# SFGLab/MultiMM

Hardware: NVIDIA B200
Metric: force_evals_per_s (higher is better)
Workload: dtype f32

## Files before the change

multimm_b200/csrc/mmm_api.cu:

```cuda
#include <math.h>
#include <string.h>

#include <algorithm>
#include <new>

#include "mmm_internal.cuh"

int mmm_launch_dots_decide(mmm_system* h);

static thread_local std::string g_create_error;
static void free_scratch(mmm_system* h);

int mmm_fail(mmm_system* h, int code, const std::string& msg) {
  if (h) h->err = msg;
  else g_create_error = msg;
  return code;
}

#define REQUIRE(h, cond, msg) \
  do { if (!(cond)) return mmm_fail((h), MMM_ERR_ARG, (msg)); } while (0)

static void derive_pair_params(mmm_system* h) {
  PairParams& p = h->pp;
  p.ev_pref = p.ev_form == MMM_EV_POWERLAW ? p.ev_eps * powf(p.ev_sigma, p.ev_power) : 0.0f;
  const float rc = p.scb_form >= 0 ? p.scb_rc : p.cob_rc;
  if (rc > 0.0f) {
    p.g_c = -1.4426950408889634f / (2.0f * rc * rc);
    p.g_inv_rc2 = 1.0f / (rc * rc);
    p.rg2 = 2.0f * rc * rc * 26.0f * 0.6931471805599453f;
  } else {
    p.g_c = 0.0f; p.g_inv_rc2 = 0.0f; p.rg2 = 0.0f;
  }
  p.cutoff2 = (float)h->cutoff * (float)h->cutoff;
}

extern "C" {

int mmm_abi_version(void) { return MMM_ABI_VERSION; }

const char* mmm_last_error(mmm_handle h) { return h ? h->err.c_str() : g_create_error.c_str(); }

int mmm_create(int device, int64_t n_beads, mmm_handle* out) {
  if (!out) return mmm_fail(nullptr, MMM_ERR_ARG, "mmm_create: out is NULL");
  *out = nullptr;
  if (n_beads < 2 || n_beads > (int64_t)1 << 24)
    return mmm_fail(nullptr, MMM_ERR_ARG, "mmm_create: n_beads must be in [2, 2^24]");
  int ndev = 0;
  cudaError_t e = cudaGetDeviceCount(&ndev);
  if (e != cudaSuccess || ndev == 0)
    return mmm_fail(nullptr, MMM_ERR_CUDA,
                    std::string("CUDA error: no usable device (") + cudaGetErrorString(e) +
                        "); this engine has no CPU fallback");
  if (device < 0 || device >= ndev) return mmm_fail(nullptr, MMM_ERR_ARG, "mmm_create: device index out of range");
  cudaDeviceProp prop;
  e = cudaGetDeviceProperties(&prop, device);
  if (e != cudaSuccess) return mmm_fail(nullptr, MMM_ERR_CUDA, std::string("CUDA error: ") + cudaGetErrorString(e));
  if (prop.major != 10)
    return mmm_fail(nullptr, MMM_ERR_CUDA,
                    "CUDA error: device is not sm_100 (B200); the kernels are built for sm_100a only");
  mmm_system* h = new (std::nothrow) mmm_system();
  if (!h) return mmm_fail(nullptr, MMM_ERR_NOMEM, "out of host memory");
  h->device = device;
  h->n = n_beads;
  h->npad = (n_beads + MMM_PAD_TO - 1) / MMM_PAD_TO * MMM_PAD_TO;
  h->ntiles = h->npad / MMM_TILE;
  h->sm_count = prop.multiProcessorCount;
  h->pp.ev_form = h->pp.cob_form = h->pp.scb_form = h->pp.chb_form = MMM_FORM_OFF;
  h->ep.sc_form = h->ep.lam_form = h->ep.cf_form = MMM_FORM_OFF;
  h->n_red_blocks = (int)((n_beads + MMM_ASM_BLOCK - 1) / MMM_ASM_BLOCK);
  h->n_dot_blocks = std::min(h->n_red_blocks, 2 * h->sm_count);
  int rc = MMM_OK;
  auto fail = [&](int code) { g_create_error = h->err; mmm_destroy(h); return code; };
  if (cudaSetDevice(device) != cudaSuccess) return fail(mmm_fail(h, MMM_ERR_CUDA, "CUDA error: cudaSetDevice"));
  if (cudaStreamCreateWithFlags(&h->stream, cudaStreamNonBlocking) != cudaSuccess)
    return fail(mmm_fail(h, MMM_ERR_CUDA, "CUDA error: cudaStreamCreate"));
  cudaEventCreate(&h->ev_a);
  cudaEventCreate(&h->ev_b);
  const size_t n3 = 3 * (size_t)n_beads;
  if ((rc = mmm_reserve(h, h->d_type, (size_t)h->npad, "bead types")) ||
      (rc = mmm_reserve(h, h->d_cstr, (size_t)n_beads, "chromosome strengths")) ||
      (rc = mmm_reserve(h, h->d_s, (size_t)n_beads, "compartment labels")) ||
      (rc = mmm_reserve(h, h->d_x, n3, "positions")) ||
      (rc = mmm_reserve(h, h->d_center, 3, "centre")) ||
      (rc = mmm_reserve(h, h->d_pos4, (size_t)h->npad, "FP32 positions")) ||
      (rc = mmm_reserve(h, h->d_soa, 3 * (size_t)h->npad, "FP32 coordinate planes")) ||
      (rc = mmm_reserve(h, h->d_tiles, (size_t)h->ntiles, "tile boxes")) ||
      (rc = mmm_reserve(h, h->d_g, n3, "gradient")) ||
      (rc = mmm_reserve(h, h->d_counter, 4, "work counters")) ||
      (rc = mmm_reserve(h, h->d_epart, (size_t)h->n_red_blocks * 6, "energy partials")) ||
      (rc = mmm_reserve(h, h->d_dpart, (size_t)h->n_red_blocks * MMM_NDOT, "dot partials")) ||
      (rc = mmm_reserve(h, h->d_eterms, MMM_NUM_TERMS, "energy terms")) ||
      (rc = mmm_reserve(h, h->d_lb, 1, "L-BFGS state")))
    return fail(rc);
  if (cudaMallocHost((void**)&h->h_done, 64) != cudaSuccess)
    return fail(mmm_fail(h, MMM_ERR_NOMEM, "CUDA error: cudaMallocHost"));
  cudaMemsetAsync(h->d_cstr, 0, sizeof(double) * n_beads, h->stream);
  cudaMemsetAsync(h->d_s, 0, n_beads, h->stream);
  cudaMemsetAsync(h->d_lb, 0, sizeof(LbfgsState), h->stream);
  std::vector<int> ty((size_t)h->npad);
  for (int64_t i = 0; i < h->npad; ++i)
    ty[i] = i < n_beads ? mmm_pack_type(0, 0) : mmm_pack_type(0, MMM_PAD_CHROM + (int)(i - n_beads));
  cudaMemcpyAsync(h->d_type, ty.data(), sizeof(int) * ty.size(), cudaMemcpyHostToDevice, h->stream);
  if (cudaStreamSynchronize(h->stream) != cudaSuccess)
    return fail(mmm_fail(h, MMM_ERR_CUDA, "CUDA error: initialisation copies failed"));
  h->types_dirty = false;
  *out = h;
  return MMM_OK;
}

int mmm_destroy(mmm_handle h) {
  if (!h) return MMM_OK;
  cudaSetDevice(h->device);
  if (h->stream) cudaStreamSynchronize(h->stream);
  mmm_dist_destroy(h);
  if (h->h_done) cudaFreeHost(h->h_done);
  for (cudaEvent_t e : h->ev_pool) cudaEventDestroy(e);
  for (cudaEvent_t e : {h->ev_a, h->ev_b, h->ev_c0, h->ev_c1, h->ct_ev0, h->ct_ev1, h->dm_ev0, h->dm_ev1,
                        h->sp_ev0, h->sp_ev1, h->lp_ev0, h->lp_ev1})
    if (e) cudaEventDestroy(e);
  if (h->stream) cudaStreamDestroy(h->stream);
  delete h;
  return MMM_OK;
}

static int check_pairs(mmm_system* h, const int32_t* i, const int32_t* j, int64_t cnt, const char* what) {
  for (int64_t q = 0; q < cnt; ++q)
    if (i[q] < 0 || j[q] < 0 || i[q] >= h->n || j[q] >= h->n || i[q] == j[q])
      return mmm_fail(h, MMM_ERR_ARG, std::string(what) + ": bead index out of range or degenerate");
  return MMM_OK;
}

int mmm_set_bonds(mmm_handle h, const int32_t* i, const int32_t* j, const double* r0, const double* k,
                  int64_t n_bonds) {
  if (!h) return MMM_ERR_ARG;
  REQUIRE(h, n_bonds >= 0 && (n_bonds == 0 || (i && j && r0 && k)), "mmm_set_bonds: NULL array");
  int rc = check_pairs(h, i, j, n_bonds, "mmm_set_bonds");
  if (rc) return rc;
  h->h_bond_i.assign(i, i + n_bonds); h->h_bond_j.assign(j, j + n_bonds);
  h->h_bond_r0.assign(r0, r0 + n_bonds); h->h_bond_k.assign(k, k + n_bonds);
  h->n_bonds = n_bonds;
  h->topo_dirty = true;
  return MMM_OK;
}

int mmm_set_loops(mmm_handle h, const int32_t* i, const int32_t* j, const double* r0, const double* k,
                  int64_t n_loops, int form) {
  if (!h) return MMM_ERR_ARG;
  REQUIRE(h, form >= MMM_LOOP_HARMONIC && form <= MMM_LOOP_GAUSSIAN_TETHER, "Unknown loop force type");
  REQUIRE(h, n_loops >= 0 && (n_loops == 0 || (i && j && r0 && k)), "mmm_set_loops: NULL array");
  int rc = check_pairs(h, i, j, n_loops, "mmm_set_loops");
  if (rc) return rc;
  h->h_loop_i.assign(i, i + n_loops); h->h_loop_j.assign(j, j + n_loops);
  h->h_loop_r0.assign(r0, r0 + n_loops); h->h_loop_k.assign(k, k + n_loops);
  h->n_loops = n_loops;
  h->loop_form = form;
  h->topo_dirty = true;
  return MMM_OK;
}

int mmm_set_angles(mmm_handle h, const int32_t* i, const int32_t* j, const int32_t* k, const double* theta0,
// ... 533 lines not shown
```

multimm_b200/csrc/mmm_internal.cuh:

```cuda
#pragma once

#include <cuda_runtime.h>
#include <stdint.h>

#include <string>
#include <vector>

#include "../../include/multimm_b200.h"

constexpr int MMM_TILE = 32;
constexpr int MMM_IBLOCK = 256;
constexpr int MMM_STAGE = 256;
constexpr int MMM_ASM_BLOCK = 128;
#ifndef MMM_LBFGS_M_VALUE
#define MMM_LBFGS_M_VALUE 6
#endif
constexpr int MMM_LBFGS_M = MMM_LBFGS_M_VALUE;
constexpr int MMM_NDOT = 6 * MMM_LBFGS_M + 7;
constexpr int MMM_PAD_TO = 512;
constexpr float MMM_PAD_COORD = 1.0e10f;
constexpr float MMM_PAD_STEP = 1.0e7f;
constexpr int MMM_PAD_CHROM = 0xFC00;

__host__ __device__ inline int mmm_pack_type(int s, int chrom) {
// ... 249 lines not shown
  cudaEvent_t dm_ev0 = nullptr, dm_ev1 = nullptr;

  bool sp_configured = false;
  double sp_rc = 0.0;
  int32_t sp_ct_bins = 0, sp_fine_bins = 0, sp_dm_bins = 0;
  DevBuf<int> d_sp_ct_bin, d_sp_fine_bin, d_sp_dm_bin;
  std::vector<int64_t> sp_dm_occ;
  int64_t sp_samples = 0;
  double sp_dm_bound = 0.0;
  float sp_ms = 0.f;
  cudaEvent_t sp_ev0 = nullptr, sp_ev1 = nullptr;
  DevBuf<unsigned long long> d_sp_map;
  DevBuf<unsigned long long> d_sp_sep;
  DevBuf<unsigned long long> d_sp_cnt;
  DevBuf<unsigned long long> d_sp_dist;
  DevBuf<long long> d_sp_tile, d_sp_table;
  DevBuf<unsigned long long> d_sp_keys[2];
  DevBuf<unsigned long long> d_sp_sval;
  DevBuf<unsigned long long> d_sp_acc_key[2], d_sp_acc_val[2];
  DevBuf<long long> d_sp_mpart;
  int64_t sp_fine_n = 0;

  bool lp_configured = false;
  double lp_rc = 0.0;
  int lp_w = 0;
  int64_t lp_rows = 0;
  int64_t lp_samples = 0;
  double lp_bound = 0.0;
  float lp_ms = 0.f;
  cudaEvent_t lp_ev0 = nullptr, lp_ev1 = nullptr;
  DevBuf<LoopRow> d_lp_row;
  DevBuf<unsigned long long> d_lp_sum;
};

struct CsSorted {
  long long keys = 0, entries = 0;
  int src = 0;
  unsigned long long cnt[2] = {0, 0};
};

int mmm_fail(mmm_system* h, int code, const std::string& msg);
#define MMM_CUDA(h, call)                                                                  \
  do {                                                                                     \
    cudaError_t _e = (call);                                                               \
    if (_e != cudaSuccess)                                                                 \
      return mmm_fail((h), MMM_ERR_CUDA,                                                   \
                      std::string("CUDA error: ") + cudaGetErrorString(_e) + " at " #call); \
  } while (0)

template <class T>
int mmm_reserve(mmm_system* h, DevBuf<T>& buf, size_t count, const char* what) {
  if (count <= buf.cap_) return MMM_OK;
  if (h && h->capturing)
    return mmm_fail(h, MMM_ERR_STATE, std::string("allocation of ") + what + " while a CUDA graph is captured");
  if (h && buf.p_) cudaStreamSynchronize(h->stream);
  buf.reset();
  cudaError_t e = cudaMalloc((void**)&buf.p_, count * sizeof(T));
  if (e != cudaSuccess) {
    buf.p_ = nullptr;
    return mmm_fail(h, MMM_ERR_NOMEM, std::string("CUDA error: ") + cudaGetErrorString(e) + " (cudaMalloc, " + what + ")");
  }
  buf.cap_ = count;
  return MMM_OK;
}

template <class T>
int mmm_upload(mmm_system* h, DevBuf<T>& buf, const std::vector<T>& v, const char* what) {
  if (v.empty()) {
    buf.reset();
    return MMM_OK;
  }
  int rc = mmm_reserve(h, buf, v.size(), what);
  if (rc) return rc;
  MMM_CUDA(h, cudaMemcpyAsync(buf, v.data(), v.size() * sizeof(T), cudaMemcpyHostToDevice, h->stream));
  MMM_CUDA(h, cudaStreamSynchronize(h->stream));
  return MMM_OK;
}

int mmm_launch_prepare(mmm_system* h, const int* d_skip);
int mmm_launch_hilbert(mmm_system* h, int p, double spacing, int32_t* d_ijk);
int mmm_launch_pair_exact(mmm_system* h, const int* d_skip, const PairParams* pp_override = nullptr);
bool mmm_pair_fast_path(const mmm_system* h);
bool mmm_pair_fast_path_pp(const PairParams& p);
bool mmm_pair_n3_eligible(const mmm_system* h);
bool mmm_pair_n3_generic(const mmm_system* h);
int mmm_n3_build_items(mmm_system* h, std::vector<int2>& items, bool chb_only);
int mmm_launch_pair_n3(mmm_system* h, const int* d_skip, bool chb_only = false);
int mmm_dist_allreduce(mmm_system* h);
void mmm_dist_destroy(mmm_system* h);
int mmm_launch_pair_n3_cut(mmm_system* h, const int* d_skip);
int mmm_cut_warp_build_items(mmm_system* h, std::vector<int2>& items);
int mmm_launch_pair_cutoff_n3(mmm_system* h, const int* d_skip);
int mmm_cutoff_resort_period();
int mmm_chb_clusters_build(mmm_system* h);
int mmm_chb_clusters_blocks(const mmm_system* h);
int mmm_launch_chb_clusters(mmm_system* h, const int* d_skip);
int mmm_launch_pair_cutoff(mmm_system* h, const int* d_skip);
int64_t mmm_cells_energy_slots(const mmm_system* h);
int mmm_upload_topology(mmm_system* h);
int mmm_upload_angles(mmm_system* h, const int32_t* ai, const int32_t* aj, const int32_t* ak,
                      const double* t0, const double* kt, int64_t na);
int mmm_launch_assemble(mmm_system* h, const int* d_skip);
int mmm_launch_finalize_energy(mmm_system* h);
int mmm_run_minimize(mmm_system* h, double tol, int64_t max_iter, mmm_min_report* out);

int mmm_contacts_dense_pass(mmm_system* h, double rc_nm, const int* d_bin, int32_t n_bins, unsigned long long* map,
                            unsigned long long* sep, unsigned long long* cnt, bool clear, cudaEvent_t ev0);
int mmm_contacts_sparse_pass(mmm_system* h, double rc_nm, const int* d_bin, int32_t n_bins, DevBuf<long long>& tile,
                             DevBuf<unsigned long long>* keys, DevBuf<long long>& table, unsigned long long* cnt,
                             cudaEvent_t ev0, cudaEvent_t ev1, CsSorted* out);
int mmm_contacts_fine_accumulate(mmm_system* h);
int mmm_contacts_fine_read(mmm_system* h, int32_t* rows_out, int32_t* cols_out, uint64_t* vals_out);
int mmm_distance_qmax(mmm_system* h, const char* who, double* dpad, double* qmax);
int mmm_distance_guard(mmm_system* h, const char* who, const std::vector<int64_t>& occ, double prior, double* bound);
int mmm_distance_pass(mmm_system* h, const int* d_bin, int32_t n_bins, unsigned long long* dmap,
                      unsigned long long* d2map, bool clear);

int mmm_evaluate(mmm_system* h, const int* d_skip);
```

multimm_b200/csrc/mmm_pair_n3.cu:

```cuda
#include <algorithm>

#include "mmm_internal.cuh"
#include "mmm_pairmath.cuh"

namespace {

constexpr int N3_THREADS = 256;
constexpr int N3_WARPS = N3_THREADS / 32;
constexpr int N3_IB = 512;
constexpr int N3_JB = 256;
constexpr int N3_STEPS = N3_JB / MMM_TILE;
constexpr double N3_FIXED = 16777216.0;
#ifndef N3_GROUP_UNROLL
#define N3_GROUP_UNROLL 2
#endif
constexpr int kGroupUnroll = N3_GROUP_UNROLL;
#ifndef N3_USE_F32X2
#define N3_USE_F32X2 1
#endif
#ifndef N3_PACKED_NEAR
#define N3_PACKED_NEAR 1
#endif
#ifndef N3_MIN_BLOCKS
#define N3_MIN_BLOCKS 2
// ... 368 lines not shown
      if (SELF) {
        live = (jl - ii) != self_d;
        i_lower = (jl - ii) > self_d;
      }
      double px = 0.0, py = 0.0, pz = 0.0;
      pairmath::pair_generic(pj, ib, (ib.w & 7) - 2, i_lower, pp, live, px, py, pz, E.gen);
      const float fx = (float)px, fy = (float)py, fz = (float)pz;
      I.fx[ii] += fx; I.fy[ii] += fy; I.fz[ii] += fz;
      ax += fx; ay += fy; az += fz;
    }
    cx[k] = ax; cy[k] = ay; cz[k] = az;
  }
}

#define N3_SHFL3(dst, src, m)                                  \
  dst##x = __shfl_xor_sync(0xffffffffu, src##x, m);            \
  dst##y = __shfl_xor_sync(0xffffffffu, src##y, m);            \
  dst##z = __shfl_xor_sync(0xffffffffu, src##z, m);

template <int EVP, int GK, int CHBM, bool SELF, bool WANT_J, bool CUT>
__device__ __forceinline__ void step64(const float4* __restrict__ sj, const JDup sjd, const int a,
                                       const int b, IBeads& I, float (&out)[3], EAcc& E, const N3Consts& c,
                                       const int* __restrict__ si4, const int self_d, const PairParams* pp = nullptr) {
  constexpr bool kPacked = N3_USE_F32X2 && GK == 0 && !SELF && (EVP > 0 ? CHBM <= 1 : CHBM == 1);
  constexpr bool kPackedNear = N3_USE_F32X2 && N3_PACKED_NEAR && GK != 0 && !SELF && EVP > 0 && CHBM <= 1;
  float s0x = 0.f, s0y = 0.f, s0z = 0.f, s1x = 0.f, s1y = 0.f, s1z = 0.f;
  float p0x = 0.f, p0y = 0.f, p0z = 0.f, p1x = 0.f, p1y = 0.f, p1z = 0.f;
#pragma unroll kGroupUnroll
  for (int g = 0; g < 4; ++g) {
    float cx[2], cy[2], cz[2];
    if constexpr (EVP < 0) pairs16_generic<SELF>(sj, a, b, 2 * g, I, cx, cy, cz, E, *pp, si4, self_d);
    else if constexpr (kPacked) pairs16_packed<EVP, CHBM, CUT>(sjd, a, b, 2 * g, I, cx, cy, cz, E, c);
    else if constexpr (kPackedNear) pairs16_packed_near<EVP, GK, CHBM, CUT>(sj, sjd, a, b, 2 * g, I, cx, cy, cz, E, c, si4);
    else pairs16<EVP, GK, CHBM, SELF, CUT>(sj, a, b, 2 * g, I, cx, cy, cz, E, c, si4, self_d);
    if (!WANT_J) continue;
    if ((g & 1) == 0) {
      s0x = cx[0]; s0y = cy[0]; s0z = cz[0];
      s1x = cx[1]; s1y = cy[1]; s1z = cz[1];
    } else {
      float t0x, t0y, t0z, t1x, t1y, t1z;
      const float c0x = cx[0], c0y = cy[0], c0z = cz[0], c1x = cx[1], c1y = cy[1], c1z = cz[1];
      N3_SHFL3(t0, c0, 8)
      N3_SHFL3(t1, c1, 8)
      t0x += s0x; t0y += s0y; t0z += s0z;
      t1x += s1x; t1y += s1y; t1z += s1z;
      if (g == 1) {
        p0x = t0x; p0y = t0y; p0z = t0z;
        p1x = t1x; p1y = t1y; p1z = t1z;
      } else {
        float u0x, u0y, u0z, u1x, u1y, u1z;
        N3_SHFL3(u0, t0, 16)
        N3_SHFL3(u1, t1, 16)
        p0x += u0x; p0y += u0y; p0z += u0z;
        p1x += u1x; p1y += u1y; p1z += u1z;
      }
    }
  }
  if (WANT_J) {
    float vx, vy, vz;
    N3_SHFL3(v, p1, 4)
    out[0] = p0x + vx; out[1] = p0y + vy; out[2] = p0z + vz;
  }
}

__device__ __forceinline__ double warp_sum_d(double v) {
#pragma unroll
  for (int o = 16; o > 0; o >>= 1) v += __shfl_xor_sync(0xffffffffu, v, o);
  return v;
}

__device__ __forceinline__ void red_fixed(unsigned long long* p, float v, double fscale, double& poison) {
  if (!(fabsf(v) <= 3.0e38f)) poison = __longlong_as_double(0x7ff8000000000000LL);
  const long long q = __double2ll_rn((double)v * fscale);
  atomicAdd(p, (unsigned long long)q);
}

__device__ __forceinline__ float box_dist2(const TileInfo& p, const TileInfo& q) {
  const float ddx = fmaxf(0.0f, fmaxf(p.lox - q.hix, q.lox - p.hix));
  const float ddy = fmaxf(0.0f, fmaxf(p.loy - q.hiy, q.loy - p.hiy));
  const float ddz = fmaxf(0.0f, fmaxf(p.loz - q.hiz, q.loz - p.hiz));
  return fmaf(ddz, ddz, fmaf(ddy, ddy, ddx * ddx));
}

template <int EVP, int GK, bool CHB, bool CUT>
__global__ void __launch_bounds__(N3_THREADS, N3_MIN_BLOCKS) k_pair_n3(const N3Args A) {
  __shared__ __align__(16) float4 s_j[2][N3_JB];
  __shared__ __align__(16) float4 s_jxy[2][N3_JB];
  __shared__ __align__(8) float2 s_jz[2][N3_JB];
  __shared__ __align__(16) TileInfo s_jt[2][N3_STEPS];
  __shared__ int s_it[N3_IB];
  __shared__ float s_acc[N3_WARPS][3][N3_JB];
  __shared__ __align__(16) double s_red[4][N3_WARPS];
  TileInfo* const s_ibox = reinterpret_cast<TileInfo*>(&s_red[0][0]);
  static_assert(sizeof(TileInfo) * N3_WARPS <= sizeof(double) * 4 * N3_WARPS, "s_ibox must fit in s_red");
  __shared__ int s_item;
  __shared__ unsigned s_mask;

  const int tid = threadIdx.x, lane = tid & 31, warp = tid >> 5;
  const int a = lane >> 2, b = lane & 3;
  const N3Consts& c = A.c;
  if (A.skip && *A.skip) return;

#pragma unroll
  for (int w = 0; w < N3_WARPS; ++w)
#pragma unroll
    for (int d = 0; d < 3; ++d) s_acc[w][d][tid] = 0.0f;

  for (;;) {
    __syncthreads();
    if (tid == 0) s_item = A.sys_counter ? atomicAdd_system(A.counter, 1) : atomicAdd(A.counter, 1);
    __syncthreads();
    const int item = A.item_first + s_item * A.item_stride;
    if (item >= A.n_items) break;
    const int2 it = A.items[item];
    const int iblk = it.x, js0 = it.y & 0xFFFFFF, cnt = it.y >> 24;
    const int64_t ibase = (int64_t)iblk * N3_IB;
    const int iw = warp * 64 + a * 8;

    IBeads I;
#pragma unroll
    for (int m = 0; m < 4; ++m) {
      const int64_t i0 = ibase + iw + 2 * m;
      I.x2[m] = *reinterpret_cast<const u64*>(A.soa + i0);
      I.y2[m] = *reinterpret_cast<const u64*>(A.soa + A.npad + i0);
      I.z2[m] = *reinterpret_cast<const u64*>(A.soa + 2 * A.npad + i0);
      I.fx[2 * m] = I.fy[2 * m] = I.fz[2 * m] = 0.0f;
      I.fx[2 * m + 1] = I.fy[2 * m + 1] = I.fz[2 * m + 1] = 0.0f;
      if (m == b) {
        s_it[iw + 2 * m] = __float_as_int(A.pos4[i0].w);
        s_it[iw + 2 * m + 1] = __float_as_int(A.pos4[i0 + 1].w);
      }
    }
    TileInfo ib = A.tiles[(ibase >> 5) + warp * 2];
    {
      const TileInfo ib2 = A.tiles[(ibase >> 5) + warp * 2 + 1];
      if (ib.cmin >= MMM_PAD_CHROM) {
        ib = ib2;
      } else if (ib2.cmin < MMM_PAD_CHROM) {
        ib.lox = fminf(ib.lox, ib2.lox); ib.loy = fminf(ib.loy, ib2.loy); ib.loz = fminf(ib.loz, ib2.loz);
        ib.hix = fmaxf(ib.hix, ib2.hix); ib.hiy = fmaxf(ib.hiy, ib2.hiy); ib.hiz = fmaxf(ib.hiz, ib2.hiz);
        ib.cmin = min(ib.cmin, ib2.cmin); ib.cmax = max(ib.cmax, ib2.cmax);
      }
    }
    const bool i_all_pad = ib.cmin >= MMM_PAD_CHROM;

    unsigned todo = cnt >= 32 ? 0xffffffffu : ((1u << cnt) - 1u);
    if (CUT) {
      if (lane == 0) s_ibox[warp] = ib;
      __syncthreads();
      if (warp == 0) {
        bool keep = false;
        if (lane < cnt) {
          const TileInfo sb = A.stage_boxes[js0 + lane];
          if (sb.cmin < MMM_PAD_CHROM) {
#pragma unroll
            for (int w = 0; w < N3_WARPS; ++w) {
              const TileInfo wb = s_ibox[w];
              keep = keep || (wb.cmin < MMM_PAD_CHROM && box_dist2(wb, sb) < c.cut2);
            }
          }
        }
        const unsigned m = __ballot_sync(0xffffffffu, keep);
        if (lane == 0) s_mask = m;
      }
      __syncthreads();
      todo = s_mask;
    }

    double de0 = 0.0, de1 = 0.0, de2 = 0.0, de3 = 0.0, poison = 0.0;

    if (todo != 0u) {
      int js = js0 + __ffs(todo) - 1;
      todo &= todo - 1u;
      {
        const float4 p0 = A.pos4[(int64_t)js * N3_JB + tid];
        s_j[0][tid] = p0;
        s_jxy[0][tid] = make_float4(-p0.x, -p0.x, -p0.y, -p0.y);
        s_jz[0][tid] = make_float2(-p0.z, -p0.z);
      }
      if (tid < 2 * N3_STEPS)
        reinterpret_cast<float4*>(s_jt[0])[tid] = reinterpret_cast<const float4*>(A.tiles + (int64_t)js * N3_STEPS)[tid];
      __syncthreads();

      for (int buf = 0;; buf ^= 1) {
        const bool more = todo != 0u;
        const int js_next = more ? js0 + __ffs(todo) - 1 : 0;
        todo &= todo - 1u;
        float4 nxt = make_float4(0.f, 0.f, 0.f, 0.f), nxt_t = nxt;
        if (more) {
          nxt = A.pos4[(int64_t)js_next * N3_JB + tid];
          if (tid < 2 * N3_STEPS)
            nxt_t = reinterpret_cast<const float4*>(A.tiles + (int64_t)js_next * N3_STEPS)[tid];
        }
        const bool diag = (js >> 1) == iblk;
        const int self_base = (int)(ibase + iw - (int64_t)js * N3_JB);
        EAcc E;
        E.ev = E.scb = E.cob = E.chb = E.cnt = 0.0f;
        E.ev2 = E.chb2 = E.cnt2 = E.scb2 = E.cob2 = pk2(0.0f, 0.0f);
        E.gen[0] = E.gen[1] = E.gen[2] = E.gen[3] = 0.0;

        if (!i_all_pad) {
          int my_class = -1;
          if (lane < N3_STEPS) {
            const TileInfo jt = s_jt[buf][lane];
            if (jt.cmin < MMM_PAD_CHROM) {
              int chb_mode = 0;
              if (CHB) {
                const bool overlap = !(ib.cmax < jt.cmin || jt.cmax < ib.cmin);
                const bool uniform = (ib.cmin == ib.cmax) && (jt.cmin == jt.cmax);
                chb_mode = overlap ? (uniform ? 1 : 2) : 0;
              }
              bool near = false;
              float d2 = 0.0f;
              if (GK != 0 || CUT) d2 = box_dist2(ib, jt);
              if (GK != 0) near = d2 < c.rg2;
              my_class = chb_mode | (near ? 4 : 0);
              if (EVP == 0 && chb_mode == 0) my_class = -1;
              if (CUT && !(d2 < c.cut2)) my_class = -1;
            }
          }
          for (int step = 0; step < N3_STEPS; ++step) {
            const int cls = __shfl_sync(0xffffffffu, my_class, step);
            if (cls < 0) continue;
            const float4* sj = s_j[buf] + step * MMM_TILE;
            const JDup sjd = {s_jxy[buf] + step * MMM_TILE, s_jz[buf] + step * MMM_TILE};
            float fj[3];
            if (diag) {
              const int self_d = self_base - step * MMM_TILE;
              step64<EVP, GK, CHB ? 2 : 0, true, false, CUT>(sj, sjd, a, b, I, fj, E, c, s_it + iw, self_d, &A.pp);
              continue;
            }
            const int chb_mode = cls & 3;
            if (cls & 4) {
              if (!CHB || chb_mode == 0) step64<EVP, GK, 0, false, true, CUT>(sj, sjd, a, b, I, fj, E, c, s_it + iw, 0, &A.pp);
              else if (chb_mode == 1) step64<EVP, GK, CHB ? 1 : 0, false, true, CUT>(sj, sjd, a, b, I, fj, E, c, s_it + iw, 0, &A.pp);
              else step64<EVP, GK, CHB ? 2 : 0, false, true, CUT>(sj, sjd, a, b, I, fj, E, c, s_it + iw, 0, &A.pp);
            } else if (!CHB || chb_mode == 0) {
              step64<EVP, 0, 0, false, true, CUT>(sj, sjd, a, b, I, fj, E, c, s_it + iw, 0, &A.pp);
            } else if (chb_mode == 1) {
              step64<EVP, 0, CHB ? 1 : 0, false, true, CUT>(sj, sjd, a, b, I, fj, E, c, s_it + iw, 0, &A.pp);
            } else {
              step64<EVP, 0, CHB ? 2 : 0, false, true, CUT>(sj, sjd, a, b, I, fj, E, c, s_it + iw, 0, &A.pp);
            }
            const int col = step * MMM_TILE + lane;
            s_acc[warp][0][col] = -fj[0];
            s_acc[warp][1][col] = -fj[1];
            s_acc[warp][2][col] = -fj[2];
          }
        }
        {
          float lo, hi;
          unpk2(E.ev2, lo, hi); E.ev += lo + hi;
          unpk2(E.chb2, lo, hi); E.chb += lo + hi;
          if (GK & 1) { unpk2(E.scb2, lo, hi); E.scb += lo + hi; }
          if (GK & 2) { unpk2(E.cob2, lo, hi); E.cob += lo + hi; }
          if (CUT) { unpk2(E.cnt2, lo, hi); E.chb = E.cnt + lo + hi; }
        }
        const double wgt = diag ? 0.5 : 1.0;
        if constexpr (EVP < 0) {
          de0 += wgt * E.gen[0]; de1 += wgt * E.gen[1]; de2 += wgt * E.gen[2]; de3 += wgt * E.gen[3];
        } else {
          de0 += wgt * (double)E.ev;
          de1 += wgt * (double)E.cob;
          de2 += wgt * (double)E.scb;
          de3 += wgt * (double)E.chb;
        }

        if (more) {
          s_j[buf ^ 1][tid] = nxt;
          s_jxy[buf ^ 1][tid] = make_float4(-nxt.x, -nxt.x, -nxt.y, -nxt.y);
          s_jz[buf ^ 1][tid] = make_float2(-nxt.z, -nxt.z);
          if (tid < 2 * N3_STEPS) reinterpret_cast<float4*>(s_jt[buf ^ 1])[tid] = nxt_t;
        }
        __syncthreads();
        if (!diag) {
          float sx = 0.0f, sy = 0.0f, sz = 0.0f;
#pragma unroll
          for (int w = 0; w < N3_WARPS; ++w) {
            sx += s_acc[w][0][tid]; sy += s_acc[w][1][tid]; sz += s_acc[w][2][tid];
            s_acc[w][0][tid] = 0.0f; s_acc[w][1][tid] = 0.0f; s_acc[w][2][tid] = 0.0f;
          }
          if (sx != 0.0f || sy != 0.0f || sz != 0.0f) {
            int64_t j = (int64_t)js * N3_JB + tid;
            if (CUT) j = A.perm[j];
            red_fixed(A.facc + j, sx, A.fscale, poison);
            red_fixed(A.facc + A.npad + j, sy, A.fscale, poison);
            red_fixed(A.facc + 2 * A.npad + j, sz, A.fscale, poison);
          }
        }
        __syncthreads();
        if (!more) break;
        js = js_next;
      }
    }

#pragma unroll
    for (int ii = 0; ii < 8; ++ii) {
      I.fx[ii] += __shfl_xor_sync(0xffffffffu, I.fx[ii], 1);
      I.fy[ii] += __shfl_xor_sync(0xffffffffu, I.fy[ii], 1);
      I.fz[ii] += __shfl_xor_sync(0xffffffffu, I.fz[ii], 1);
      I.fx[ii] += __shfl_xor_sync(0xffffffffu, I.fx[ii], 2);
      I.fy[ii] += __shfl_xor_sync(0xffffffffu, I.fy[ii], 2);
      I.fz[ii] += __shfl_xor_sync(0xffffffffu, I.fz[ii], 2);
    }
#pragma unroll
    for (int ii = 0; ii < 8; ++ii) {
      if ((ii >> 1) == b) {
        int64_t i = ibase + iw + ii;
        if (CUT) {
          if (I.fx[ii] == 0.0f && I.fy[ii] == 0.0f && I.fz[ii] == 0.0f) continue;
          i = A.perm[i];
        }
        red_fixed(A.facc + i, I.fx[ii], A.fscale, poison);
        red_fixed(A.facc + A.npad + i, I.fy[ii], A.fscale, poison);
        red_fixed(A.facc + 2 * A.npad + i, I.fz[ii], A.fscale, poison);
      }
    }

    de0 = de0 * A.e_ev + poison;
    de1 *= A.e_gauss;
    de2 *= A.e_gauss;
    if (!CUT) de3 *= A.e_chb;
    de0 = warp_sum_d(de0); de1 = warp_sum_d(de1); de2 = warp_sum_d(de2); de3 = warp_sum_d(de3);
    if (lane == 0) { s_red[0][warp] = de0; s_red[1][warp] = de1; s_red[2][warp] = de2; s_red[3][warp] = de3; }
    __syncthreads();
    if (tid < 4) {
      double s = 0.0;
#pragma unroll
      for (int w = 0; w < N3_WARPS; ++w) s += s_red[tid][w];
      if (CUT && tid == 3) {
        A.npairs[item] = s;
        s = 0.0;
      }
      A.epair[(size_t)item * 4 + tid] = s;
    }
  }
}

constexpr double CW_EFIXED = 1048576.0;
constexpr int CW_CHUNK = 8;

struct CutWArgs {
  const float4* pos4;
  const float* soa;
  const TileInfo* tiles;
  const TileInfo* stage_boxes;
  const int* perm;
  unsigned long long* facc;
  long long* eacc;
  const int2* items;
  int* counter;
  const int* skip;
  int64_t npad;
  int nstages, item_begin, item_end;
  double fscale, e_ev, e_gauss;
  N3Consts c;
};

template <int EVP, int GK>
__global__ void __launch_bounds__(N3_THREADS, N3_MIN_BLOCKS) k_pair_cut_warp(const CutWArgs A) {
  __shared__ __align__(16) float4 s_j[N3_WARPS][MMM_TILE];
  __shared__ __align__(16) float4 s_jxy[N3_WARPS][MMM_TILE];
  __shared__ __align__(8) float2 s_jz[N3_WARPS][MMM_TILE];
  __shared__ int s_it[N3_WARPS][64];
  const int lane = threadIdx.x & 31, warp = threadIdx.x >> 5;
  const int a = lane >> 2, b = lane & 3;
  const N3Consts& c = A.c;
  if (A.skip && *A.skip) return;

  for (;;) {
    int item = 0;
    if (lane == 0) item = A.item_begin + atomicAdd(A.counter, 1);
    item = __shfl_sync(0xffffffffu, item, 0);
    if (item >= A.item_end) break;
    const int2 it = A.items[item];
    const int g = it.x, s0 = it.y, s1 = min(s0 + CW_CHUNK, A.nstages);
    const int64_t ibase = (int64_t)g * 64;
    IBeads I;
    __syncwarp();
#pragma unroll
    for (int m = 0; m < 4; ++m) {
      const int64_t i0 = ibase + 8 * a + 2 * m;
      I.x2[m] = *reinterpret_cast<const u64*>(A.soa + i0);
      I.y2[m] = *reinterpret_cast<const u64*>(A.soa + A.npad + i0);
      I.z2[m] = *reinterpret_cast<const u64*>(A.soa + 2 * A.npad + i0);
      I.fx[2 * m] = I.fy[2 * m] = I.fz[2 * m] = 0.0f;
      I.fx[2 * m + 1] = I.fy[2 * m + 1] = I.fz[2 * m + 1] = 0.0f;
      if (m == b) {
        s_it[warp][8 * a + 2 * m] = __float_as_int(A.pos4[i0].w);
        s_it[warp][8 * a + 2 * m + 1] = __float_as_int(A.pos4[i0 + 1].w);
      }
    }
    TileInfo ib = A.tiles[2 * g];
    {
      const TileInfo ib2 = A.tiles[2 * g + 1];
      if (ib.cmin >= MMM_PAD_CHROM) {
        ib = ib2;
      } else if (ib2.cmin < MMM_PAD_CHROM) {
        ib.lox = fminf(ib.lox, ib2.lox); ib.loy = fminf(ib.loy, ib2.loy); ib.loz = fminf(ib.loz, ib2.loz);
        ib.hix = fmaxf(ib.hix, ib2.hix); ib.hiy = fmaxf(ib.hiy, ib2.hiy); ib.hiz = fmaxf(ib.hiz, ib2.hiz);
      }
    }
    if (ib.cmin >= MMM_PAD_CHROM) continue;
    __syncwarp();

    bool keep = false;
    if (s0 + lane < s1) {
      const TileInfo sb = A.stage_boxes[s0 + lane];
      keep = sb.cmin < MMM_PAD_CHROM && box_dist2(ib, sb) < c.cut2;
    }
    unsigned smask = __ballot_sync(0xffffffffu, keep);
    double de0 = 0.0, de1 = 0.0, de2 = 0.0, de3 = 0.0, poison = 0.0;

    while (smask) {
      const int s = s0 + __ffs(smask) - 1;
      smask &= smask - 1u;
      int cls = -1;
      if (lane < N3_STEPS) {
        const int t = s * N3_STEPS + lane;
// ... 42 lines not shown
          float lo, hi;
          unpk2(E.ev2, lo, hi); E.ev += lo + hi;
          if (GK & 1) { unpk2(E.scb2, lo, hi); E.scb += lo + hi; }
          if (GK & 2) { unpk2(E.cob2, lo, hi); E.cob += lo + hi; }
          unpk2(E.cnt2, lo, hi); E.cnt += lo + hi;
        }
        de0 += wgt * (double)E.ev;
        de1 += wgt * (double)E.cob;
        de2 += wgt * (double)E.scb;
        de3 += wgt * (double)E.cnt;
        __syncwarp();
      }
    }

#pragma unroll
    for (int ii = 0; ii < 8; ++ii) {
      I.fx[ii] += __shfl_xor_sync(0xffffffffu, I.fx[ii], 1);
      I.fy[ii] += __shfl_xor_sync(0xffffffffu, I.fy[ii], 1);
      I.fz[ii] += __shfl_xor_sync(0xffffffffu, I.fz[ii], 1);
      I.fx[ii] += __shfl_xor_sync(0xffffffffu, I.fx[ii], 2);
      I.fy[ii] += __shfl_xor_sync(0xffffffffu, I.fy[ii], 2);
      I.fz[ii] += __shfl_xor_sync(0xffffffffu, I.fz[ii], 2);
    }
#pragma unroll
    for (int ii = 0; ii < 8; ++ii) {
      if ((ii >> 1) == b && (I.fx[ii] != 0.0f || I.fy[ii] != 0.0f || I.fz[ii] != 0.0f)) {
        const int64_t i = A.perm[ibase + 8 * a + ii];
        red_fixed(A.facc + i, I.fx[ii], A.fscale, poison);
        red_fixed(A.facc + A.npad + i, I.fy[ii], A.fscale, poison);
        red_fixed(A.facc + 2 * A.npad + i, I.fz[ii], A.fscale, poison);
      }
    }
    de0 = warp_sum_d(de0 * A.e_ev + poison);
    de1 = warp_sum_d(de1 * A.e_gauss);
    de2 = warp_sum_d(de2 * A.e_gauss);
    de3 = warp_sum_d(de3);
    if (lane < 4) {
      const double v = lane == 0 ? de0 : (lane == 1 ? de1 : (lane == 2 ? de2 : de3));
      const long long fx = isfinite(v) ? __double2ll_rn(v * CW_EFIXED) : 0x7fffffffffffffffLL;
      if (fx != 0) atomicAdd(reinterpret_cast<unsigned long long*>(A.eacc + lane), (unsigned long long)fx);
    }
  }
}

__global__ void k_cut_finish(long long* __restrict__ eacc, double* __restrict__ epair_slot, double* __restrict__ npairs,
                             const int* __restrict__ skip) {
  if (skip && *skip) return;
  const int t = threadIdx.x;
  if (t < 4) {
    const long long v = eacc[t];
    eacc[t] = 0;
    const double d = v == 0x7fffffffffffffffLL ? __longlong_as_double(0x7ff8000000000000LL) : (double)v / CW_EFIXED;
    if (t < 3) epair_slot[t] = d;
    else { npairs[0] = d; epair_slot[3] = 0.0; }
  }
}

template <int EVP, int GK>
int launch_cut_warp(mmm_system* h, const CutWArgs& A) {
  int occ = 1;
  cudaOccupancyMaxActiveBlocksPerMultiprocessor(&occ, k_pair_cut_warp<EVP, GK>, N3_THREADS, 0);
  if (occ < 1) occ = 1;
  int grid = h->sm_count * occ;
  const int n_local = A.item_end - A.item_begin;
  if (grid * N3_WARPS > n_local) grid = (n_local + N3_WARPS - 1) / N3_WARPS;
  if (grid < 1) grid = 1;
  k_pair_cut_warp<EVP, GK><<<grid, N3_THREADS, 0, h->stream>>>(A);
  return 0;
}

template <int EVP>
int launch_cut_warp_gk(mmm_system* h, const CutWArgs& A, int gk) {
  switch (gk) {
    case 0: return launch_cut_warp<EVP, 0>(h, A);
    case 1: return launch_cut_warp<EVP, 1>(h, A);
    case 2: return launch_cut_warp<EVP, 2>(h, A);
    default: return launch_cut_warp<EVP, 3>(h, A);
  }
}

template <int EVP, int GK, bool CHB, bool CUT>
int launch_n3(mmm_system* h, const N3Args& A) {
  int occ = 1;
  cudaOccupancyMaxActiveBlocksPerMultiprocessor(&occ, k_pair_n3<EVP, GK, CHB, CUT>, N3_THREADS, 0);
  if (occ < 1) occ = 1;
  int grid = h->sm_count * occ;
  const int n_local = (A.n_items - A.item_first + A.item_stride - 1) / A.item_stride;
  if (grid > n_local) grid = n_local > 0 ? n_local : 1;
  k_pair_n3<EVP, GK, CHB, CUT><<<grid, N3_THREADS, 0, h->stream>>>(A);
  return 0;
}

template <int EVP>
int launch_n3_evp(mmm_system* h, const N3Args& A, int gk, bool chb) {
  switch (gk * 2 + (chb ? 1 : 0)) {
    case 0: return launch_n3<EVP, 0, false, false>(h, A);
    case 1: return launch_n3<EVP, 0, true, false>(h, A);
    case 2: return launch_n3<EVP, 1, false, false>(h, A);
    case 3: return launch_n3<EVP, 1, true, false>(h, A);
    case 4: return launch_n3<EVP, 2, false, false>(h, A);
    case 5: return launch_n3<EVP, 2, true, false>(h, A);
    case 6: return launch_n3<EVP, 3, false, false>(h, A);
    default: return launch_n3<EVP, 3, true, false>(h, A);
  }
}

template <int EVP>
int launch_n3_cut(mmm_system* h, const N3Args& A, int gk) {
  switch (gk) {
    case 0: return launch_n3<EVP, 0, false, true>(h, A);
    case 1: return launch_n3<EVP, 1, false, true>(h, A);
    case 2: return launch_n3<EVP, 2, false, true>(h, A);
    default: return launch_n3<EVP, 3, false, true>(h, A);
  }
}

void fill_consts(const PairParams& p, bool chb_only, bool with_chb, N3Args& A) {
  const double U = chb_only ? 1.0 : (double)p.ev_power * (double)p.ev_eps * pow((double)p.ev_sigma, (double)p.ev_power);
  A.pp = p;
  A.fscale = U * N3_FIXED;
  A.e_ev = chb_only ? 0.0 : (double)p.ev_eps * pow((double)p.ev_sigma, (double)p.ev_power);
  N3Consts& c = A.c;
  c.ev_rs = p.ev_rs;
  c.g_c = p.g_c;
  c.rg2 = p.rg2;
  c.chb_kc = p.chb_kc;
  c.chb_c = (with_chb && p.chb_form >= 0) ? (float)((double)p.chb_de / U) : 0.0f;
  c.gk = chb_only ? 0 : ((p.scb_form >= 0 ? 1 : 0) | (p.cob_form >= 0 ? 2 : 0));
  c.cut2 = p.cutoff2;
  const double rc = p.scb_form >= 0 ? p.scb_rc : p.cob_rc;
  const double inv = rc > 0.0 ? 1.0 / (rc * rc * U) : 0.0;
  c.a_scb[0] = (float)(p.scb_e[3] * inv);
  c.a_scb[1] = (float)(p.scb_e[2] * inv);
  c.a_scb[2] = 0.0f;
  c.a_scb[3] = (float)(p.scb_e[1] * inv);
  c.a_scb[4] = (float)(p.scb_e[0] * inv);
  c.a_cob[0] = 0.0f;
  c.a_cob[1] = (float)(p.cob_ea * inv);
  c.a_cob[2] = (float)(p.cob_eb * inv);
  c.a_cob[3] = 0.0f;
  A.e_gauss = -(rc * rc) * U;
  A.e_chb = (double)p.chb_de;
}

}

bool mmm_pair_n3_eligible(const mmm_system* h) {
  if (!mmm_pair_fast_path(h)) return false;
  if (h->pp.ev_form != MMM_EV_POWERLAW) return false;
  if (!(h->pp.ev_eps > 0.0f) || !(h->pp.ev_sigma > 0.0f)) return false;
  return true;
}

bool mmm_pair_n3_generic(const mmm_system* h) {
  const PairParams& p = h->pp;
  const bool any = p.ev_form >= 0 || p.cob_form >= 0 || p.scb_form >= 0 || p.chb_form >= 0;
  return any && !mmm_pair_fast_path(h);
}

int mmm_n3_build_items(mmm_system* h, std::vector<int2>& items, bool chb_only) {
  const int64_t nib = h->npad / N3_IB, njs = h->npad / N3_JB;
  std::vector<int> lo((size_t)njs, 0x7fffffff), hi((size_t)njs, -1);
  if (chb_only) {
    for (int64_t i = 0; i < h->n; ++i) {
      const int c = h->h_chrom.empty() ? 0 : h->h_chrom[(size_t)i];
      const int64_t s = i / N3_JB;
      lo[s] = std::min(lo[s], c);
      hi[s] = std::max(hi[s], c);
    }
  }
  auto wanted = [&](int64_t ib, int64_t js) {
    if (!chb_only) return true;
    if ((js >> 1) == ib) return hi[js] >= 0;
    const int ilo = std::min(lo[2 * ib], lo[2 * ib + 1]), ihi = std::max(hi[2 * ib], hi[2 * ib + 1]);
    return hi[js] >= 0 && ihi >= 0 && !(ihi < lo[js] || hi[js] < ilo);
  };
  int64_t pairs = 0;
  for (int64_t i = 0; i < nib; ++i)
    for (int64_t js = 2 * i; js < njs; ++js) pairs += wanted(i, js) ? 1 : 0;
  const int64_t target_items = (int64_t)h->sm_count * 2 * 48;
  int64_t cj = pairs / target_items;
  cj = cj < 1 ? 1 : (cj > 16 ? 16 : cj);
  items.clear();
  for (int64_t i = 0; i < nib; ++i) {
    int64_t js = 2 * i;
    while (js < njs) {
      if (!wanted(i, js)) { ++js; continue; }
      int64_t cnt = 1;
      while (cnt < cj && js + cnt < njs && wanted(i, js + cnt)) ++cnt;
      items.push_back(make_int2((int)i, (int)(js | (cnt << 24))));
      js += cnt;
    }
  }
  if (items.empty()) items.push_back(make_int2(0, 0));
  return MMM_OK;
}

int mmm_launch_pair_n3(mmm_system* h, const int* d_skip, bool chb_only) {
  const PairParams& p = h->pp;
  N3Args A;
  A.pos4 = h->d_pos4;
  A.soa = h->d_soa;
  A.tiles = h->d_tiles;
  A.facc = h->d_facc;
  A.epair = h->d_epair;
  A.items = h->d_items;
  A.counter = h->d_counter;
  A.skip = d_skip;
  A.npad = h->npad;
  A.n_items = h->n3_items;
  A.stage_boxes = nullptr;
  A.perm = nullptr;
  A.npairs = nullptr;
  A.sys_counter = 0;
  fill_consts(p, chb_only, true, A);
  const bool generic = !chb_only && !mmm_pair_n3_eligible(h);
  if (generic) {
    A.fscale = N3_FIXED;
    A.e_ev = A.e_gauss = A.e_chb = 1.0;
  }
  const N3Consts& c = A.c;

  const bool timed = !chb_only;
  const bool collect = timed && h->ev_cursor >= 0 && (size_t)(2 * h->ev_cursor + 1) < h->ev_pool.size();
  cudaEvent_t ea = collect ? h->ev_pool[2 * h->ev_cursor] : h->ev_a;
  cudaEvent_t eb = collect ? h->ev_pool[2 * h->ev_cursor + 1] : h->ev_b;
  if (collect) h->ev_cursor++;
  if (timed && !h->capturing) MMM_CUDA(h, cudaEventRecord(ea, h->stream));
// ... 116 lines not shown
```

Baseline: 61.20.

## Double-buffer column accumulators and prefetch j-blocks with cp.async in n3 pair kernel

The column-force accumulator moves to dynamic shared memory and is double-buffered, so the reduction and atomic emission of one j-block is deferred and overlapped with computing the next, which removes one __syncthreads per step. The next j-block's positions and tile boxes are now fetched straight into shared memory with cp.async instead of being staged through registers. The dynamic shared memory footprint doubles the accumulator space, which needs an opt-in attribute at init and may lower occupancy. Optional clock64 phase profiling is added behind a compile flag.

```diff
diff --git a/multimm_b200/csrc/mmm_api.cu b/multimm_b200/csrc/mmm_api.cu
--- a/multimm_b200/csrc/mmm_api.cu
+++ b/multimm_b200/csrc/mmm_api.cu
@@ -76,6 +76,7 @@
     return fail(mmm_fail(h, MMM_ERR_CUDA, "CUDA error: cudaStreamCreate"));
   cudaEventCreate(&h->ev_a);
   cudaEventCreate(&h->ev_b);
+  if ((rc = mmm_pair_n3_init(h))) return fail(rc);
   const size_t n3 = 3 * (size_t)n_beads;
   if ((rc = mmm_reserve(h, h->d_type, (size_t)h->npad, "bead types")) ||
       (rc = mmm_reserve(h, h->d_cstr, (size_t)n_beads, "chromosome strengths")) ||
diff --git a/multimm_b200/csrc/mmm_internal.cuh b/multimm_b200/csrc/mmm_internal.cuh
--- a/multimm_b200/csrc/mmm_internal.cuh
+++ b/multimm_b200/csrc/mmm_internal.cuh
@@ -355,6 +355,7 @@
 int mmm_launch_pair_exact(mmm_system* h, const int* d_skip, const PairParams* pp_override = nullptr);
 bool mmm_pair_fast_path(const mmm_system* h);
 bool mmm_pair_fast_path_pp(const PairParams& p);
+int mmm_pair_n3_init(mmm_system* h);
 bool mmm_pair_n3_eligible(const mmm_system* h);
 bool mmm_pair_n3_generic(const mmm_system* h);
 int mmm_n3_build_items(mmm_system* h, std::vector<int2>& items, bool chb_only);
diff --git a/multimm_b200/csrc/mmm_pair_n3.cu b/multimm_b200/csrc/mmm_pair_n3.cu
--- a/multimm_b200/csrc/mmm_pair_n3.cu
+++ b/multimm_b200/csrc/mmm_pair_n3.cu
@@ -474,6 +474,47 @@
   return fmaf(ddz, ddz, fmaf(ddy, ddy, ddx * ddx));
 }
 
+#ifdef N3_PHASES
+enum N3Phase { PH_FAR, PH_TILES, PH_DIAG, PH_COLS, PH_BARRIER, PH_EMIT, PH_ITEM, PH_QUEUE, PH_NEXT, N3_NPHASES };
+__device__ unsigned long long g_n3_phases[N3_NPHASES];
+#define N3_PHASE(k)                                                                   \
+  do {                                                                                \
+    const long long t_ = clock64();                                                   \
+    if (lane == 0) s_ph[warp][k] += (unsigned long long)(t_ - ph_t);                  \
+    ph_t = t_;                                                                        \
+  } while (0)
+#else
+#define N3_PHASE(k) \
+  do {              \
+  } while (0)
+#endif
+
+constexpr size_t N3_DYN_SMEM = sizeof(float) * 2 * N3_WARPS * 3 * N3_JB;
+typedef float N3Cols[N3_WARPS][3][N3_JB];
+
+__device__ __forceinline__ void cp_async16(void* smem, const void* gmem) {
+  const unsigned s = (unsigned)__cvta_generic_to_shared(smem);
+  asm volatile("cp.async.cg.shared.global [%0], [%1], 16;" ::"r"(s), "l"(gmem) : "memory");
+}
+__device__ __forceinline__ void cp_async_wait_all() { asm volatile("cp.async.wait_all;" ::: "memory"); }
+
+template <bool CUT>
+__device__ __forceinline__ void emit_columns(N3Cols& col, const int js, const int tid, const N3Args& A, double& poison) {
+  float sx = 0.0f, sy = 0.0f, sz = 0.0f;
+#pragma unroll
+  for (int w = 0; w < N3_WARPS; ++w) {
+    sx += col[w][0][tid]; sy += col[w][1][tid]; sz += col[w][2][tid];
+    col[w][0][tid] = 0.0f; col[w][1][tid] = 0.0f; col[w][2][tid] = 0.0f;
+  }
+  if (sx != 0.0f || sy != 0.0f || sz != 0.0f) {
+    int64_t j = (int64_t)js * N3_JB + tid;
+    if (CUT) j = A.perm[j];
+    red_fixed(A.facc + j, sx, A.fscale, poison);
+    red_fixed(A.facc + A.npad + j, sy, A.fscale, poison);
+    red_fixed(A.facc + 2 * A.npad + j, sz, A.fscale, poison);
+  }
+}
+
 template <int EVP, int GK, bool CHB, bool CUT>
 __global__ void __launch_bounds__(N3_THREADS, N3_MIN_BLOCKS) k_pair_n3(const N3Args A) {
   __shared__ __align__(16) float4 s_j[2][N3_JB];
@@ -481,8 +522,9 @@
   __shared__ __align__(8) float2 s_jz[2][N3_JB];
   __shared__ __align__(16) TileInfo s_jt[2][N3_STEPS];
   __shared__ int s_it[N3_IB];
-  __shared__ float s_acc[N3_WARPS][3][N3_JB];
   __shared__ __align__(16) double s_red[4][N3_WARPS];
+  extern __shared__ __align__(16) float n3_dyn[];
+  N3Cols* const s_acc = reinterpret_cast<N3Cols*>(n3_dyn);
   TileInfo* const s_ibox = reinterpret_cast<TileInfo*>(&s_red[0][0]);
   static_assert(sizeof(TileInfo) * N3_WARPS <= sizeof(double) * 4 * N3_WARPS, "s_ibox must fit in s_red");
   __shared__ int s_item;
@@ -492,16 +534,25 @@
   const int a = lane >> 2, b = lane & 3;
   const N3Consts& c = A.c;
   if (A.skip && *A.skip) return;
-
-#pragma unroll
-  for (int w = 0; w < N3_WARPS; ++w)
-#pragma unroll
-    for (int d = 0; d < 3; ++d) s_acc[w][d][tid] = 0.0f;
+#ifdef N3_PHASES
+  __shared__ unsigned long long s_ph[N3_WARPS][N3_NPHASES];
+  if (lane == 0)
+    for (int k = 0; k < N3_NPHASES; ++k) s_ph[warp][k] = 0ull;
+  long long ph_t = clock64();
+#endif
+
+#pragma unroll
+  for (int w = 0; w < 2 * N3_WARPS; ++w)
+#pragma unroll
+    for (int d = 0; d < 3; ++d) s_acc[w >> 3][w & 7][d][tid] = 0.0f;
+  int abuf = 0;
 
   for (;;) {
     __syncthreads();
+    N3_PHASE(PH_BARRIER);
     if (tid == 0) s_item = A.sys_counter ? atomicAdd_system(A.counter, 1) : atomicAdd(A.counter, 1);
     __syncthreads();
+    N3_PHASE(PH_QUEUE);
     const int item = A.item_first + s_item * A.item_stride;
     if (item >= A.n_items) break;
     const int2 it = A.items[item];
@@ -573,17 +624,20 @@
       if (tid < 2 * N3_STEPS)
         reinterpret_cast<float4*>(s_jt[0])[tid] = reinterpret_cast<const float4*>(A.tiles + (int64_t)js * N3_STEPS)[tid];
       __syncthreads();
+      N3_PHASE(PH_ITEM);
+      int pend_js = -1;
 
       for (int buf = 0;; buf ^= 1) {
         const bool more = todo != 0u;
         const int js_next = more ? js0 + __ffs(todo) - 1 : 0;
         todo &= todo - 1u;
-        float4 nxt = make_float4(0.f, 0.f, 0.f, 0.f), nxt_t = nxt;
         if (more) {
-          nxt = A.pos4[(int64_t)js_next * N3_JB + tid];
+          cp_async16(&s_j[buf ^ 1][tid], A.pos4 + (int64_t)js_next * N3_JB + tid);
           if (tid < 2 * N3_STEPS)
-            nxt_t = reinterpret_cast<const float4*>(A.tiles + (int64_t)js_next * N3_STEPS)[tid];
-        }
+            cp_async16(reinterpret_cast<float4*>(s_jt[buf ^ 1]) + tid,
+                       reinterpret_cast<const float4*>(A.tiles + (int64_t)js_next * N3_STEPS) + tid);
+        }
+        N3_PHASE(PH_NEXT);
         const bool diag = (js >> 1) == iblk;
         const int self_base = (int)(ibase + iw - (int64_t)js * N3_JB);
         EAcc E;
@@ -611,6 +665,7 @@
               if (CUT && !(d2 < c.cut2)) my_class = -1;
             }
           }
+          N3Cols& cols = s_acc[abuf];
           for (int step = 0; step < N3_STEPS; ++step) {
             const int cls = __shfl_sync(0xffffffffu, my_class, step);
             if (cls < 0) continue;
@@ -620,6 +675,7 @@
             if (diag) {
               const int self_d = self_base - step * MMM_TILE;
               step64<EVP, GK, CHB ? 2 : 0, true, false, CUT>(sj, sjd, a, b, I, fj, E, c, s_it + iw, self_d, &A.pp);
+              N3_PHASE(PH_DIAG);
               continue;
             }
             const int chb_mode = cls & 3;
@@ -627,17 +683,22 @@
               if (!CHB || chb_mode == 0) step64<EVP, GK, 0, false, true, CUT>(sj, sjd, a, b, I, fj, E, c, s_it + iw, 0, &A.pp);
               else if (chb_mode == 1) step64<EVP, GK, CHB ? 1 : 0, false, true, CUT>(sj, sjd, a, b, I, fj, E, c, s_it + iw, 0, &A.pp);
               else step64<EVP, GK, CHB ? 2 : 0, false, true, CUT>(sj, sjd, a, b, I, fj, E, c, s_it + iw, 0, &A.pp);
+              N3_PHASE(PH_TILES);
             } else if (!CHB || chb_mode == 0) {
               step64<EVP, 0, 0, false, true, CUT>(sj, sjd, a, b, I, fj, E, c, s_it + iw, 0, &A.pp);
+              N3_PHASE(PH_FAR);
             } else if (chb_mode == 1) {
               step64<EVP, 0, CHB ? 1 : 0, false, true, CUT>(sj, sjd, a, b, I, fj, E, c, s_it + iw, 0, &A.pp);
+              N3_PHASE(PH_FAR);
             } else {
               step64<EVP, 0, CHB ? 2 : 0, false, true, CUT>(sj, sjd, a, b, I, fj, E, c, s_it + iw, 0, &A.pp);
+              N3_PHASE(PH_TILES);
             }
             const int col = step * MMM_TILE + lane;
-            s_acc[warp][0][col] = -fj[0];
-            s_acc[warp][1][col] = -fj[1];
-            s_acc[warp][2][col] = -fj[2];
+            cols[warp][0][col] = -fj[0];
+            cols[warp][1][col] = -fj[1];
+            cols[warp][2][col] = -fj[2];
+            N3_PHASE(PH_COLS);
           }
         }
         {
@@ -657,33 +718,30 @@
           de2 += wgt * (double)E.scb;
           de3 += wgt * (double)E.chb;
         }
-
+        N3_PHASE(PH_ITEM);
+
+        if (pend_js >= 0) emit_columns<CUT>(s_acc[abuf ^ 1], pend_js, tid, A, poison);
+        N3_PHASE(PH_EMIT);
+        if (!diag) {
+          pend_js = js;
+          abuf ^= 1;
+        } else {
+          pend_js = -1;
+        }
         if (more) {
-          s_j[buf ^ 1][tid] = nxt;
-          s_jxy[buf ^ 1][tid] = make_float4(-nxt.x, -nxt.x, -nxt.y, -nxt.y);
-          s_jz[buf ^ 1][tid] = make_float2(-nxt.z, -nxt.z);
-          if (tid < 2 * N3_STEPS) reinterpret_cast<float4*>(s_jt[buf ^ 1])[tid] = nxt_t;
-        }
+          cp_async_wait_all();
+          const float4 p = s_j[buf ^ 1][tid];
+          s_jxy[buf ^ 1][tid] = make_float4(-p.x, -p.x, -p.y, -p.y);
+          s_jz[buf ^ 1][tid] = make_float2(-p.z, -p.z);
+        }
+        N3_PHASE(PH_NEXT);
         __syncthreads();
-        if (!diag) {
-          float sx = 0.0f, sy = 0.0f, sz = 0.0f;
-#pragma unroll
-          for (int w = 0; w < N3_WARPS; ++w) {
-            sx += s_acc[w][0][tid]; sy += s_acc[w][1][tid]; sz += s_acc[w][2][tid];
-            s_acc[w][0][tid] = 0.0f; s_acc[w][1][tid] = 0.0f; s_acc[w][2][tid] = 0.0f;
-          }
-          if (sx != 0.0f || sy != 0.0f || sz != 0.0f) {
-            int64_t j = (int64_t)js * N3_JB + tid;
-            if (CUT) j = A.perm[j];
-            red_fixed(A.facc + j, sx, A.fscale, poison);
-            red_fixed(A.facc + A.npad + j, sy, A.fscale, poison);
-            red_fixed(A.facc + 2 * A.npad + j, sz, A.fscale, poison);
-          }
-        }
-        __syncthreads();
+        N3_PHASE(PH_BARRIER);
         if (!more) break;
         js = js_next;
       }
+      if (pend_js >= 0) emit_columns<CUT>(s_acc[abuf ^ 1], pend_js, tid, A, poison);
+      N3_PHASE(PH_EMIT);
     }
 
 #pragma unroll
@@ -726,7 +784,12 @@
       }
       A.epair[(size_t)item * 4 + tid] = s;
     }
-  }
+    N3_PHASE(PH_ITEM);
+  }
+#ifdef N3_PHASES
+  if (lane == 0)
+    for (int k = 0; k < N3_NPHASES; ++k) atomicAdd(&g_n3_phases[k], s_ph[warp][k]);
+#endif
 }
 
 constexpr double CW_EFIXED = 1048576.0;
@@ -935,13 +998,30 @@
 template <int EVP, int GK, bool CHB, bool CUT>
 int launch_n3(mmm_system* h, const N3Args& A) {
   int occ = 1;
-  cudaOccupancyMaxActiveBlocksPerMultiprocessor(&occ, k_pair_n3<EVP, GK, CHB, CUT>, N3_THREADS, 0);
+  cudaOccupancyMaxActiveBlocksPerMultiprocessor(&occ, k_pair_n3<EVP, GK, CHB, CUT>, N3_THREADS, N3_DYN_SMEM);
   if (occ < 1) occ = 1;
   int grid = h->sm_count * occ;
   const int n_local = (A.n_items - A.item_first + A.item_stride - 1) / A.item_stride;
   if (grid > n_local) grid = n_local > 0 ? n_local : 1;
-  k_pair_n3<EVP, GK, CHB, CUT><<<grid, N3_THREADS, 0, h->stream>>>(A);
+  k_pair_n3<EVP, GK, CHB, CUT><<<grid, N3_THREADS, N3_DYN_SMEM, h->stream>>>(A);
   return 0;
+}
+
+template <int EVP, int GK, bool CHB, bool CUT>
+cudaError_t allow_n3_smem() {
+  return cudaFuncSetAttribute(k_pair_n3<EVP, GK, CHB, CUT>, cudaFuncAttributeMaxDynamicSharedMemorySize, (int)N3_DYN_SMEM);
+}
+
+template <int EVP>
+cudaError_t allow_n3_smem_evp() {
+  const cudaError_t e[] = {
+      allow_n3_smem<EVP, 0, false, false>(), allow_n3_smem<EVP, 0, true, false>(), allow_n3_smem<EVP, 1, false, false>(),
+      allow_n3_smem<EVP, 1, true, false>(),  allow_n3_smem<EVP, 2, false, false>(), allow_n3_smem<EVP, 2, true, false>(),
+      allow_n3_smem<EVP, 3, false, false>(), allow_n3_smem<EVP, 3, true, false>(),  allow_n3_smem<EVP, 0, false, true>(),
+      allow_n3_smem<EVP, 1, false, true>(),  allow_n3_smem<EVP, 2, false, true>(),  allow_n3_smem<EVP, 3, false, true>()};
+  for (cudaError_t x : e)
+    if (x != cudaSuccess) return x;
+  return cudaSuccess;
 }
 
 template <int EVP>
@@ -997,6 +1077,24 @@
 }
 
 }
+
+int mmm_pair_n3_init(mmm_system* h) {
+  cudaError_t e = allow_n3_smem_evp<6>();
+  if (e == cudaSuccess) e = allow_n3_smem_evp<3>();
+  if (e == cudaSuccess) e = allow_n3_smem<0, 0, true, false>();
+  if (e == cudaSuccess) e = allow_n3_smem<-1, 0, false, false>();
+  if (e != cudaSuccess) return mmm_fail(h, MMM_ERR_CUDA, std::string("CUDA error: k_pair_n3 shared memory: ") + cudaGetErrorString(e));
+  return MMM_OK;
+}
+
+#ifdef N3_PHASES
+extern "C" int mmm_n3_phases_take(unsigned long long* out) {
+  if (cudaDeviceSynchronize() != cudaSuccess) return 1;
+  if (cudaMemcpyFromSymbol(out, g_n3_phases, sizeof(unsigned long long) * N3_NPHASES) != cudaSuccess) return 1;
+  const unsigned long long zero[N3_NPHASES] = {};
+  return cudaMemcpyToSymbol(g_n3_phases, zero, sizeof(zero)) == cudaSuccess ? 0 : 1;
+}
+#endif
 
 bool mmm_pair_n3_eligible(const mmm_system* h) {
   if (!mmm_pair_fast_path(h)) return false;
```

Measured after the change: 62.48 (median of 6 runs). 2.1% higher.
